# facebookresearch/vsc2022

Hardware: AMD Instinct MI355X
Metric: query-videos localized/sec @ 512-d SSCD (higher is better)
Workload: dtype fp32 results; int8 / fp16 MFMA pre-filters; 1 GPU; BASELINE configs[3]: full pipeline incl. score normalisation + TN localisation, 40000 query videos split over 1 GPU(s), 2000000 reference + 2000000 noise frames; query_videos_per_gpu=40000, query_frames_per_gpu=1000000, ref_frames=2000000, dim=512, global_k=48000000, candidates=1000000, pairs_localized=200000, matches=446939, hits=48000000, score_normalisation_in_step=True, parallelism=single GPU

## Files before the change

### vsc2022_amd/csrc/api_aux.hip

```cpp
#include "api_internal.h"

extern "C" {


struct DeviceCtx {
    hipStream_t stream = nullptr;
    hipStream_t own_stream = nullptr;
    Workspace ws;
    std::mutex mu;
};
static DeviceCtx* device_ctx(int device) {
    static std::mutex g_mu;
    static std::vector<DeviceCtx*> ctxs;
    std::lock_guard<std::mutex> lk(g_mu);
    if ((int)ctxs.size() <= device) ctxs.resize(device + 1, nullptr);
    if (!ctxs[device]) {
        DeviceCtx* c = new DeviceCtx();
        if (hipStreamCreateWithFlags(&c->own_stream, hipStreamNonBlocking) != hipSuccess) {
            delete c;
            return nullptr;
        }
        c->stream = c->own_stream;
        ctxs[device] = c;
    }
// ... 39 lines not shown
    VSC_TRY(check_device(device));
    VSC_HIP(hipSetDevice(device));
    DeviceCtx* c = device_ctx(device);
    if (!c) {
        set_error("vsc_pair_max: cannot create device context");
        return VSC_ERR_HIP;
    }
    std::lock_guard<std::mutex> lk(c->mu);
    Workspace& ws = c->ws;
    const void *di, *dj, *ds, *dq, *dr;
    VSC_TRY(to_device(hit_i, (size_t)n * 4, hits_mem, ws.hA[0], &di, c->stream));
    VSC_TRY(to_device(hit_j, (size_t)n * 4, hits_mem, ws.hA[1], &dj, c->stream));
    VSC_TRY(to_device(hit_s, (size_t)n * 4, hits_mem, ws.hA[2], &ds, c->stream));
    VSC_TRY(to_device(row2q, (size_t)nq_rows * 4, maps_mem, ws.maps0, &dq, c->stream));
    VSC_TRY(to_device(row2r, (size_t)nr_rows * 4, maps_mem, ws.maps1, &dr, c->stream));
    int32_t *oq = out_q, *orr = out_r;
    float* os = out_s;
    int64_t* of = out_first;
    const int64_t ocap = out_mem == VSC_MEM_HOST ? n : cap;
    if (out_mem == VSC_MEM_HOST) {
        VSC_TRY(ws.out[0].reserve((size_t)n * 4));
        VSC_TRY(ws.out[1].reserve((size_t)n * 4));
        VSC_TRY(ws.out[2].reserve((size_t)n * 4));
        VSC_TRY(ws.out[3].reserve((size_t)n * 8));
        oq = ws.out[0].as<int32_t>();
        orr = ws.out[1].as<int32_t>();
        os = ws.out[2].as<float>();
        of = ws.out[3].as<int64_t>();
    }
    int64_t np = 0;
    AuxTimer tm;
    tm.begin(0, c->stream);
    VSC_TRY(pair_max_device((const int32_t*)di, (const int32_t*)dj, (const float*)ds, n, (const int32_t*)dq,
                            (const int32_t*)dr, nq_rows, nr_rows, ws.w0, ws.w1, ws.w2, ws.w3, ws.tmp, ws.cnt, oq, orr, os, of,
                            ocap, &np, c->stream));
    tm.end(12.0 * (double)n + 20.0 * (double)np, c->stream);
    *n_pairs = np;
    if (out_mem == VSC_MEM_HOST) {
        if (np > cap) {
            set_error("vsc_pair_max: output capacity %lld < %lld pairs", (long long)cap, (long long)np);
            return VSC_ERR_CAPACITY;
        }
        VSC_HIP(hipMemcpyAsync(out_q, oq, (size_t)np * 4, hipMemcpyDeviceToHost, c->stream));
        VSC_HIP(hipMemcpyAsync(out_r, orr, (size_t)np * 4, hipMemcpyDeviceToHost, c->stream));
        VSC_HIP(hipMemcpyAsync(out_s, os, (size_t)np * 4, hipMemcpyDeviceToHost, c->stream));
        if (out_first) VSC_HIP(hipMemcpyAsync(out_first, of, (size_t)np * 8, hipMemcpyDeviceToHost, c->stream));
    }
    VSC_HIP(hipStreamSynchronize(c->stream));
    tm.collect();
    return VSC_OK;
}

int vsc_sort_hits(const int32_t* hit_i, const int32_t* hit_j, const float* hit_s, int64_t n, int hits_mem, int64_t max_row,
                  int64_t max_ref, int32_t* out_i, int32_t* out_j, float* out_s, int out_mem, int device) {
    if (n < 0 || (n > 0 && (!hit_i || !hit_j || !hit_s || !out_i || !out_j || !out_s))) {
        set_error("vsc_sort_hits: invalid argument");
        return VSC_ERR_INVALID;
    }
    if (n == 0) return VSC_OK;
    VSC_TRY(check_device(device));
    VSC_HIP(hipSetDevice(device));
    DeviceCtx* c = device_ctx(device);
    if (!c) {
        set_error("vsc_sort_hits: cannot create device context");
        return VSC_ERR_HIP;
    }
    std::lock_guard<std::mutex> lk(c->mu);
    Workspace& ws = c->ws;
    const void *di, *dj, *ds;
    VSC_TRY(to_device(hit_i, (size_t)n * 4, hits_mem, ws.hA[0], &di, c->stream));
    VSC_TRY(to_device(hit_j, (size_t)n * 4, hits_mem, ws.hA[1], &dj, c->stream));
    VSC_TRY(to_device(hit_s, (size_t)n * 4, hits_mem, ws.hA[2], &ds, c->stream));
    int32_t *oi = out_i, *oj = out_j;
    float* os = out_s;
    if (out_mem == VSC_MEM_HOST) {
        for (int k = 0; k < 3; ++k) VSC_TRY(ws.out[k].reserve((size_t)n * 4));
        oi = ws.out[0].as<int32_t>();
        oj = ws.out[1].as<int32_t>();
        os = ws.out[2].as<float>();
    }
    const int64_t all = (int64_t)1 << 31;
    int64_t m = 0;
    VSC_TRY(sort_hits_topk((const int32_t*)di, (const int32_t*)dj, (const float*)ds, n, n, max_row > 0 ? max_row : all,
                           max_ref > 0 ? max_ref : all, ws.w0, ws.w1, ws.w2, ws.w3, ws.tmp, oi, oj, os, 0, &m, c->stream));
    if (out_mem == VSC_MEM_HOST) {
        VSC_HIP(hipMemcpyAsync(out_i, oi, (size_t)n * 4, hipMemcpyDeviceToHost, c->stream));
        VSC_HIP(hipMemcpyAsync(out_j, oj, (size_t)n * 4, hipMemcpyDeviceToHost, c->stream));
        VSC_HIP(hipMemcpyAsync(out_s, os, (size_t)n * 4, hipMemcpyDeviceToHost, c->stream));
    }
    VSC_HIP(hipStreamSynchronize(c->stream));
    return VSC_OK;
}

int vsc_score_histogram(const float* scores, int64_t n, const int64_t* state, int shift, int64_t* hist, int device) {
    if (n < 0 || (n > 0 && !scores) || !state || !hist || (shift != 0 && shift != 8 && shift != 16 && shift != 24)) {
        set_error("vsc_score_histogram: invalid argument");
        return VSC_ERR_INVALID;
    }
    VSC_TRY(check_device(device));
    VSC_HIP(hipSetDevice(device));
    DeviceCtx* c = device_ctx(device);
    if (!c) {
        set_error("vsc_score_histogram: cannot create device context");
        return VSC_ERR_HIP;
    }
    std::lock_guard<std::mutex> lk(c->mu);
    VSC_TRY(launch_score_hist(scores, (long long)n, reinterpret_cast<const long long*>(state), shift,
                              reinterpret_cast<long long*>(hist), c->stream));
    if (c->stream == c->own_stream) VSC_HIP(hipStreamSynchronize(c->stream));
    return VSC_OK;
}

int vsc_score_pick(const int64_t* hist, int64_t* state, int shift, int device) {
    if (!hist || !state || (shift != 0 && shift != 8 && shift != 16 && shift != 24)) {
        set_error("vsc_score_pick: invalid argument");
        return VSC_ERR_INVALID;
    }
    VSC_TRY(check_device(device));
    VSC_HIP(hipSetDevice(device));
    DeviceCtx* c = device_ctx(device);
    if (!c) {
        set_error("vsc_score_pick: cannot create device context");
        return VSC_ERR_HIP;
    }
    std::lock_guard<std::mutex> lk(c->mu);
    VSC_TRY(launch_score_pick(reinterpret_cast<const long long*>(hist), reinterpret_cast<long long*>(state), shift, c->stream));
    if (c->stream == c->own_stream) VSC_HIP(hipStreamSynchronize(c->stream));
    return VSC_OK;
}

int vsc_filter_hits(const int32_t* hit_i, const int32_t* hit_j, const float* hit_s, int64_t n, float radius, int32_t* out_i,
                    int32_t* out_j, float* out_s, int64_t* n_out, int device) {
    if (n < 0 || !n_out || (n > 0 && (!hit_i || !hit_j || !hit_s || !out_i || !out_j || !out_s)) || !(radius == radius)) {
        set_error("vsc_filter_hits: invalid argument");
        return VSC_ERR_INVALID;
    }
    *n_out = 0;
    if (n == 0) return VSC_OK;
    VSC_TRY(check_device(device));
    VSC_HIP(hipSetDevice(device));
    DeviceCtx* c = device_ctx(device);
    if (!c) {
        set_error("vsc_filter_hits: cannot create device context");
        return VSC_ERR_HIP;
    }
    std::lock_guard<std::mutex> lk(c->mu);
    VSC_TRY(c->ws.cnt.reserve(sizeof(unsigned long long)));
    VSC_TRY(launch_filter_hits(hit_i, hit_j, hit_s, (long long)n, radius, out_i, out_j, out_s, c->ws.cnt.as<unsigned long long>(),
                               c->stream));
    unsigned long long kept = 0;
    VSC_HIP(hipMemcpyAsync(&kept, c->ws.cnt.p, sizeof(kept), hipMemcpyDeviceToHost, c->stream));
    VSC_HIP(hipStreamSynchronize(c->stream));
    *n_out = (int64_t)kept;
    return VSC_OK;
}

int vsc_argsort_scores(const float* scores, int64_t n, int mem, int32_t* perm, int perm_mem, int device) {
    if (n < 0 || (n > 0 && (!scores || !perm))) {
        set_error("vsc_argsort_scores: invalid argument");
        return VSC_ERR_INVALID;
    }
    if (n == 0) return VSC_OK;
    VSC_TRY(check_device(device));
    VSC_HIP(hipSetDevice(device));
    DeviceCtx* c = device_ctx(device);
    if (!c) {
        set_error("vsc_argsort_scores: cannot create device context");
// ... 416 lines not shown
```

### vsc2022_amd/csrc/kernels.h

```cpp
#pragma once
#include "vscmi_common.h"
#include "cand_list.h"

namespace vscmi {

struct SimThreshArgs {
    const float* Q; const float* R; int dpad; int nq; int i0; int nr; int tq; int tr;
    const float* radius; int32_t* out_i; int32_t* out_j; float* out_s;
    unsigned long long* counter; long long cap; int* overflow;
};
struct SimF16Args {
    const _Float16* Q; const _Float16* R;
    const float* qn; const float* rn;
    int dpadh; int nq; int i0; int nr; int tq; int tr;
    float c1, c2, c3;
    const float* radius; int32_t* out_i; int32_t* out_j;
    const float* row_thr;
    int seg_cap; int* seg_count; int64_t tail_base; long long tail_cap; int tail_shift; int* tail_fill; unsigned long long* tail_count;
    int* overflow;
};
constexpr int F16P_PANEL_ROWS = 128;
constexpr int F16P_COL_STEP = 512;
constexpr int F16P_MAX_DPADH = 512;
struct SimF16PArgs {
// ... 59 lines not shown
    unsigned long long* n_cand_total;
    const int* overflow;
};
struct SimKnnArgs {
    const float* Q; const float* R; int dpad; int nq; int nr; int tq; int tr; int nchunk; int k;
    float* part_s; int32_t* part_j;
    int no_first_tile_select;
};
struct KnnMergeArgs {
    const float* part_s; const int32_t* part_j; int nq; int nchunk; int k; float* out_s; int64_t* out_j; int l2;
};
struct ScoreMatArgs { const float* Q; const float* R; int dpad; int dim; int nq; int nr; int metric; float* S; };
struct MatThreshArgs {
    const float* S; int nq; int nr; int i0; const float* radius; int32_t* out_i; int32_t* out_j; float* out_s;
    unsigned long long* counter; long long cap; int* overflow;
};
struct MatKnnArgs { const float* S; int nq; int nr; int k; float* part_s; int32_t* part_j; };
struct SelectCtl {
    unsigned long long n; unsigned long long n_tmp; float radius; int overflow; int active;
    unsigned int prefix; unsigned int prefix_mask; unsigned long long rank; unsigned int hist[256];
    unsigned long long n_rethreshold;
    unsigned long long n_cand_total;
    unsigned long long n_tail;
};
struct TnPairArgs {
    const float* qfeat; const float* rfeat; const int64_t* q_off; const int64_t* r_off; int dpad;
    const int32_t* pair_q; const int32_t* pair_r; const int32_t* work; int n_work; vsc_tn_params prm;
    float bias; int max_lq; int lds_tile_floats; float* slab; int64_t slab_floats;
    int32_t* out_nbox; int32_t* out_boxes; float* out_boxmax;
    const float* sims_in; const int64_t* sims_off; const int32_t* sims_lq; const int32_t* sims_lr;
    char* state; int64_t state_bytes;
};
struct TnSimsArgs { const float* qfeat; const float* rfeat; int64_t qrow0, rrow0; int lq, lr, dpad; float bias; float* out; };

int launch_sim_thresh(const SimThreshArgs&, hipStream_t);
int launch_sim_f16(const SimF16Args&, hipStream_t);
int sim_f16_grid(int tq, int tr);
int launch_rescore(const RescoreArgs&, hipStream_t);
int launch_cand_count(const RescoreArgs&, int, unsigned long long*, hipStream_t);
int launch_cand_compact(const RescoreArgs&, int, uint32_t*, uint32_t*, unsigned long long*, hipStream_t);
int launch_rescore_dense(const RescoreArgs&, const uint32_t*, const uint32_t*, long long, hipStream_t,
                         const unsigned long long* n_dev = nullptr);
int launch_f16_screen(const ScreenArgs&, hipStream_t);
int sort_candidates_by_ref(uint32_t*, uint32_t*, uint32_t*, uint32_t*, int64_t, int64_t, DevBuf&, const uint32_t**,
                           const uint32_t**, hipStream_t);
void sim_f16p_plan(int64_t nq, int64_t nr, int* npanel, int* nsteps, int* slice, int* grid);
int launch_sim_f16p(const SimF16PArgs&, int grid, hipStream_t);
int launch_sim_i8p(const SimI8PArgs&, int grid, hipStream_t);
bool sim_i8p_pairs(int dpad8, int npanel, int nsteps, int slice, bool force);
int launch_quant_ref_frag(const float*, int, void*, float4*, int64_t, int64_t, int, const ExcludedDims&, const float*, hipStream_t);
int launch_col_sums(const float*, int64_t, int, double*, double*, hipStream_t);
int launch_row_center(const float*, int, int, const float*, float*, float*, hipStream_t);
int launch_dim_minmax(const float*, int64_t, int, unsigned*, unsigned*, hipStream_t);
int launch_meta_looseness(const float4*, int64_t, double*, hipStream_t);
int launch_quant_query_panels(const float*, int, int, int, void*, int, float4*, const int32_t*, const float*, float*,
                              const ExcludedDims&, hipStream_t);
int launch_row_absmax(const float*, int, int, const ExcludedDims&, float*, hipStream_t);
int launch_row_bias_thresholds(const float*, int, int, const float*, const float*, const ExcludedDims&, const float*, const float*, float*,
                               hipStream_t);
int sort_rows_by_threshold(const float*, int64_t, DevBuf&, DevBuf&, DevBuf&, DevBuf&, DevBuf&, const int32_t**, hipStream_t);
int argsort_scores_desc(const float*, int64_t, DevBuf&, DevBuf&, DevBuf&, DevBuf&, DevBuf&, const int32_t**, hipStream_t);
int launch_ctl_init(SelectCtl*, float, hipStream_t);
int launch_filter_hits(const int32_t*, const int32_t*, const float*, long long, float, int32_t*, int32_t*, float*, unsigned long long*,
                       hipStream_t);
int launch_score_hist(const float*, long long, const long long*, int, long long*, hipStream_t);
int launch_score_pick(const long long*, long long*, int, hipStream_t);
int launch_merge_topk(const float*, const long long*, long long, int, int, float*, long long*, hipStream_t);
int sort_rows_by_threshold_then_scale(const float*, const float*, int64_t, int, DevBuf&, DevBuf&, DevBuf&, DevBuf&, DevBuf&,
                                      const int32_t**, hipStream_t);
int launch_pack_half_frag(const float*, int64_t, int, _Float16*, float*, int64_t, int64_t, int, hipStream_t);
int launch_pack_half(const float*, int64_t, int, _Float16*, float*, int64_t, int, hipStream_t);
int launch_sim_knn(const SimKnnArgs&, hipStream_t);
int launch_knn_merge(const KnnMergeArgs&, hipStream_t);
int knn_from_hits(const int32_t*, const int32_t*, const float*, int64_t, int64_t, int, DevBuf&, DevBuf&, DevBuf&,
                  DevBuf&, DevBuf&, float*, int64_t*, hipStream_t);
int launch_knn_row_thr(const float*, int64_t, int, float*, int64_t, hipStream_t);
int launch_knn_seed_hits(const float*, const int64_t*, int64_t, int, int32_t*, int32_t*, float*, unsigned long long*, hipStream_t);
int launch_score_matrix(const ScoreMatArgs&, hipStream_t);
int launch_matrix_thresh(const MatThreshArgs&, hipStream_t);
int launch_matrix_knn(const MatKnnArgs&, hipStream_t);
int set_thresh_kernel_attrs();
int enqueue_rethreshold(SelectCtl*, int32_t*, int32_t*, float*, int32_t*, int32_t*, float*, unsigned long long, hipStream_t);
int sort_hits_topk(const int32_t*, const int32_t*, const float*, int64_t, int64_t, int64_t, int64_t, DevBuf&, DevBuf&,
                   DevBuf&, DevBuf&, DevBuf&, int32_t*, int32_t*, float*, int, int64_t*, hipStream_t);
int sort_hits_rowcol(const int32_t*, const int32_t*, const float*, int64_t, DevBuf&, DevBuf&, DevBuf&, DevBuf&,
                     DevBuf&, int32_t*, int32_t*, float*, int, hipStream_t);
int pair_max_device(const int32_t*, const int32_t*, const float*, int64_t, const int32_t*, const int32_t*, int64_t, int64_t,
                    DevBuf&, DevBuf&, DevBuf&, DevBuf&, DevBuf&, DevBuf&, int32_t*, int32_t*, float*, int64_t*,
                    int64_t, int64_t*, hipStream_t);
int launch_pack_rows(const float*, int64_t, int, float*, int64_t, int, hipStream_t);
int launch_row_normalize(const float*, int64_t, int, float*, hipStream_t);
size_t tn_state_bytes_host(int, int, int, int idx_bytes = 2);
int launch_tn_pairs(const TnPairArgs&, size_t, hipStream_t);
int launch_tn_sims(const TnSimsArgs&, hipStream_t);
int launch_encode_rows(const void*, bool, int64_t, int, _Float16*, float*, int64_t, int64_t, int, bool, int*, hipStream_t);
int launch_decode_rows(const _Float16*, int, bool, int64_t, int64_t, int64_t, float*, int, bool, hipStream_t);
int launch_unpack_rows(const float*, int, int64_t, int, float*, hipStream_t);
int launch_half_to_float(const _Float16*, int64_t, float*, hipStream_t);
int launch_score_matrix_h16(const ScoreMatArgs&, const _Float16*, int, bool, hipStream_t);
int launch_hits_mark(const unsigned long long*, unsigned long long*, hipStream_t);
int launch_hits_add_offset(int32_t*, const unsigned long long*, const unsigned long long*, long long, int, hipStream_t);
int launch_knn_parts_scatter(const float*, const int32_t*, int64_t, int, int, int, int, int, float*, int32_t*, hipStream_t);


}
```

### vsc2022_amd/csrc/radix.h

```cpp
#pragma once
#include "vscmi_common.h"

namespace vscmi {

constexpr int RADIX_ITEMS = 16;
constexpr int RADIX_TILE = 256 * RADIX_ITEMS;

template <class K>
__device__ __forceinline__ unsigned radix_digit(K key, int shift, bool desc) {
    if (desc) key = ~key;
    return (unsigned)(key >> shift) & 255u;
}

template <class K>
__global__ __launch_bounds__(256) void radix_hist_kernel(const K* __restrict__ keys, int64_t n, int shift, bool desc,
                                                         unsigned* __restrict__ hist, int ntiles) {
    __shared__ unsigned h[256];
    h[threadIdx.x] = 0;
    __syncthreads();
    const int64_t base = (int64_t)blockIdx.x * RADIX_TILE;
#pragma unroll 4
    for (int k = 0; k < RADIX_ITEMS; ++k) {
        const int64_t e = base + k * 256 + threadIdx.x;
        if (e < n) atomicAdd(&h[radix_digit(keys[e], shift, desc)], 1u);
    }
    __syncthreads();
    hist[(int64_t)threadIdx.x * ntiles + blockIdx.x] = h[threadIdx.x];
}

__global__ __launch_bounds__(256) void radix_scan_rows_kernel(unsigned* __restrict__ hist, int ntiles,
                                                              unsigned* __restrict__ totals) {
    __shared__ unsigned part[256];
    unsigned* row = hist + (int64_t)blockIdx.x * ntiles;
    const int per = (ntiles + 255) / 256;
    const int t0 = threadIdx.x * per;
    unsigned s = 0;
    for (int t = t0; t < min(ntiles, t0 + per); ++t) s += row[t];
    part[threadIdx.x] = s;
    __syncthreads();
    for (int off = 1; off < 256; off <<= 1) {
        const unsigned v = threadIdx.x >= off ? part[threadIdx.x - off] : 0u;
        __syncthreads();
        part[threadIdx.x] += v;
        __syncthreads();
    }
    unsigned run = threadIdx.x ? part[threadIdx.x - 1] : 0u;
    for (int t = t0; t < min(ntiles, t0 + per); ++t) {
        const unsigned c = row[t];
        row[t] = run;
        run += c;
    }
    if (threadIdx.x == 255) totals[blockIdx.x] = part[255];
}

__global__ __launch_bounds__(256) void radix_scan_totals_kernel(unsigned* __restrict__ totals) {
    __shared__ unsigned part[256];
    part[threadIdx.x] = totals[threadIdx.x];
    __syncthreads();
    for (int off = 1; off < 256; off <<= 1) {
        const unsigned v = threadIdx.x >= off ? part[threadIdx.x - off] : 0u;
        __syncthreads();
        part[threadIdx.x] += v;
        __syncthreads();
    }
    totals[threadIdx.x] = threadIdx.x ? part[threadIdx.x - 1] : 0u;
}

template <class K, class V>
__global__ __launch_bounds__(256) void radix_scatter_kernel(const K* __restrict__ keys_in, const V* __restrict__ vals_in,
                                                            K* __restrict__ keys_out, V* __restrict__ vals_out, int64_t n,
                                                            int shift, bool desc, const unsigned* __restrict__ hist,
                                                            const unsigned* __restrict__ totals, int ntiles) {
    __shared__ unsigned wcount[4][256];
    __shared__ unsigned dstart[256];
    __shared__ unsigned gbase[256];
    __shared__ K skey[RADIX_TILE];
    __shared__ V sval[RADIX_TILE];
    const int lane = threadIdx.x & 63, wave = threadIdx.x >> 6;
    for (int x = threadIdx.x; x < 4 * 256; x += 256) (&wcount[0][0])[x] = 0;
    gbase[threadIdx.x] = totals[threadIdx.x] + hist[(int64_t)threadIdx.x * ntiles + blockIdx.x];
    __syncthreads();
    const int64_t tile0 = (int64_t)blockIdx.x * RADIX_TILE;
    const int64_t base = tile0 + (int64_t)wave * (RADIX_ITEMS * 64);
    K key[RADIX_ITEMS];
    unsigned rank[RADIX_ITEMS];
#pragma unroll
    for (int k = 0; k < RADIX_ITEMS; ++k) {
        const int64_t e = base + k * 64 + lane;
        const bool valid = e < n;
        key[k] = valid ? keys_in[e] : (K)0;
        const unsigned d = radix_digit(key[k], shift, desc);
        unsigned long long peers = __ballot(valid);
#pragma unroll
        for (int b = 0; b < 8; ++b) {
            const unsigned long long m = __ballot((d >> b) & 1u);
            peers &= ((d >> b) & 1u) ? m : ~m;
        }
        const unsigned before = (unsigned)__popcll(peers & ((1ull << lane) - 1));
        unsigned c = 0;
        if (valid) c = wcount[wave][d];
        __builtin_amdgcn_wave_barrier();
        if (valid && before == 0) wcount[wave][d] = c + (unsigned)__popcll(peers);
        __builtin_amdgcn_wave_barrier();
        rank[k] = c + before;
    }
    __syncthreads();
    {
        const int d = threadIdx.x;
        unsigned run = 0;
#pragma unroll
        for (int w = 0; w < 4; ++w) {
            const unsigned c = wcount[w][d];
            wcount[w][d] = run;
            run += c;
        }
        dstart[d] = run;
    }
    __syncthreads();
    for (int off = 1; off < 256; off <<= 1) {
        const unsigned v = threadIdx.x >= off ? dstart[threadIdx.x - off] : 0u;
        __syncthreads();
        dstart[threadIdx.x] += v;
        __syncthreads();
    }
    const unsigned mine_incl = dstart[threadIdx.x];
    const unsigned prev_incl = threadIdx.x ? dstart[threadIdx.x - 1] : 0u;
    __syncthreads();
    dstart[threadIdx.x] = prev_incl;
    (void)mine_incl;
    __syncthreads();
#pragma unroll
    for (int k = 0; k < RADIX_ITEMS; ++k) {
        const int64_t e = base + k * 64 + lane;
        if (e < n) {
            const unsigned d = radix_digit(key[k], shift, desc);
            const unsigned slot = dstart[d] + wcount[wave][d] + rank[k];
            skey[slot] = key[k];
            sval[slot] = vals_in[e];
        }
    }
    __syncthreads();
    const int cnt = (int)min((int64_t)RADIX_TILE, n - tile0);
#pragma unroll 4
    for (int k = 0; k < RADIX_ITEMS; ++k) {
        const int slot = k * 256 + threadIdx.x;
        if (slot < cnt) {
            const K kk = skey[slot];
            const unsigned d = radix_digit(kk, shift, desc);
            const int64_t pos = (int64_t)gbase[d] + (slot - dstart[d]);
            keys_out[pos] = kk;
            vals_out[pos] = sval[slot];
        }
    }
}

inline size_t radix_tmp_bytes(int64_t n) {
    const int64_t ntiles = (n + RADIX_TILE - 1) / RADIX_TILE;
    return (size_t)(256 * ntiles + 256) * sizeof(unsigned);
}

template <class K, class V>
int radix_sort_pairs(K* keys_a, K* keys_b, V* vals_a, V* vals_b, int64_t n, int begin_bit, int end_bit, bool desc,
                     void* tmp, hipStream_t stream, int begin2 = 0, int end2 = 0) {
    if (n <= 0) return 0;
    if (n > 0xffffffffLL) {
        set_error("radix_sort_pairs: %lld entries exceed the 2^32 limit of the sort", (long long)n);
        return -1;
    }
    const int ntiles = (int)((n + RADIX_TILE - 1) / RADIX_TILE);
    unsigned* hist = reinterpret_cast<unsigned*>(tmp);
    unsigned* totals = hist + (size_t)256 * ntiles;
    int where = 0;
    for (int pass = 0;; ++pass) {
        const int n1 = (end_bit - begin_bit + 7) / 8;
        const int shift = pass < n1 ? begin_bit + 8 * pass : begin2 + 8 * (pass - n1);
        if (pass >= n1 && shift >= end2) break;
        const K* ki = where ? keys_b : keys_a;
        const V* vi = where ? vals_b : vals_a;
        K* ko = where ? keys_a : keys_b;
        V* vo = where ? vals_a : vals_b;
        hipLaunchKernelGGL((radix_hist_kernel<K>), dim3((unsigned)ntiles), dim3(256), 0, stream, ki, n, shift, desc, hist, ntiles);
        hipLaunchKernelGGL(radix_scan_rows_kernel, dim3(256), dim3(256), 0, stream, hist, ntiles, totals);
        hipLaunchKernelGGL(radix_scan_totals_kernel, dim3(1), dim3(256), 0, stream, totals);
        hipLaunchKernelGGL((radix_scatter_kernel<K, V>), dim3((unsigned)ntiles), dim3(256), 0, stream, ki, vi, ko, vo, n, shift,
                           desc, hist, totals, ntiles);
        if (hipGetLastError() != hipSuccess) return -1;
        where ^= 1;
    }
    return where;
}

}
```

### vsc2022_amd/csrc/sortpairs.hip

```cpp
#include <cfloat>
#include <cstring>
#include <utility>

#include "kernels.h"
#include "radix.h"

namespace vscmi {

__global__ __launch_bounds__(256) void pack_hits_kernel(const int32_t* i, const int32_t* j,
                                                        const float* s, int64_t n, uint64_t* key64,
                                                        uint32_t* key32) {
    const int64_t x = (int64_t)blockIdx.x * 256 + threadIdx.x;
    if (x >= n) return;
    key64[x] = ((uint64_t)(uint32_t)i[x] << 32) | (uint32_t)j[x];
    key32[x] = f2key(s[x]);
}

__global__ __launch_bounds__(256) void unpack_hits_kernel(const uint64_t* key64, const uint32_t* key32,
                                                          int64_t n, int32_t* i, int32_t* j, float* s,
                                                          int negate) {
    const int64_t x = (int64_t)blockIdx.x * 256 + threadIdx.x;
    if (x >= n) return;
    i[x] = (int32_t)(key64[x] >> 32);
    j[x] = (int32_t)(key64[x] & 0xffffffffu);
    const float v = key2f(key32[x]);
    s[x] = negate ? -v : v;
}

static inline unsigned grid_for(int64_t n) { return (unsigned)((n + 255) / 256); }

static int bits_for(uint64_t maxval) {
    int b = 1;
    while (b < 64 && (maxval >> b)) ++b;
    return b;
}

int sort_hits_topk(const int32_t* hi, const int32_t* hj, const float* hs, int64_t n, int64_t K,
                   int64_t max_i, int64_t max_j, DevBuf& w0, DevBuf& w1, DevBuf& w2, DevBuf& w3, DevBuf& tmp,
                   int32_t* out_i, int32_t* out_j, float* out_s, int negate, int64_t* n_out,
                   hipStream_t stream) {
    const int64_t m = n < K ? n : K;
    *n_out = m;
    if (n <= 0) return VSC_OK;
    VSC_TRY(w0.reserve(sizeof(uint64_t) * n));
    VSC_TRY(w1.reserve(sizeof(uint64_t) * n));
    VSC_TRY(w2.reserve(sizeof(uint32_t) * n));
    VSC_TRY(w3.reserve(sizeof(uint32_t) * n));
    uint64_t* k64a = w0.as<uint64_t>();
    uint64_t* k64b = w1.as<uint64_t>();
    uint32_t* k32a = w2.as<uint32_t>();
    uint32_t* k32b = w3.as<uint32_t>();
    hipLaunchKernelGGL(pack_hits_kernel, dim3(grid_for(n)), dim3(256), 0, stream, hi, hj, hs, n, k64a, k32a);
    VSC_HIP(hipGetLastError());
    const int end_bit = 32 + bits_for((uint64_t)(max_i > 0 ? max_i : 1));
    VSC_TRY(tmp.reserve(radix_tmp_bytes(n)));
    int w = radix_sort_pairs<uint64_t, uint32_t>(k64a, k64b, k32a, k32b, n, 0, max_j > 0 ? bits_for((uint64_t)max_j) : 32, false,
                                                 tmp.p, stream, 32, end_bit);
    if (w < 0) { set_error("radix sort launch failed"); return VSC_ERR_HIP; }
    if (w) { std::swap(k64a, k64b); std::swap(k32a, k32b); }
    w = radix_sort_pairs<uint32_t, uint64_t>(k32a, k32b, k64a, k64b, n, 0, 32, true, tmp.p, stream);
    if (w < 0) { set_error("radix sort launch failed"); return VSC_ERR_HIP; }
    if (w) { std::swap(k64a, k64b); std::swap(k32a, k32b); }
    hipLaunchKernelGGL(unpack_hits_kernel, dim3(grid_for(m)), dim3(256), 0, stream, k64a, k32a, m, out_i, out_j, out_s, negate);
    VSC_HIP(hipGetLastError());
    return VSC_OK;
}

__global__ __launch_bounds__(256) void thr_keys_kernel(const float* __restrict__ thr, int n, uint32_t* __restrict__ keys,
                                                       int32_t* __restrict__ vals) {
    const int x = blockIdx.x * 256 + threadIdx.x;
    if (x >= n) return;
    keys[x] = f2key(thr[x]);
    vals[x] = x;
}

int sort_rows_by_threshold(const float* thr, int64_t n, DevBuf& w0, DevBuf& w1, DevBuf& w2, DevBuf& w3, DevBuf& tmp,
                           const int32_t** perm, hipStream_t stream) {
    *perm = nullptr;
    if (n <= 0) return VSC_OK;
    VSC_TRY(w0.reserve(sizeof(uint32_t) * n));
    VSC_TRY(w1.reserve(sizeof(uint32_t) * n));
    VSC_TRY(w2.reserve(sizeof(int32_t) * n));
    VSC_TRY(w3.reserve(sizeof(int32_t) * n));
    VSC_TRY(tmp.reserve(radix_tmp_bytes(n)));
    uint32_t *ka = w0.as<uint32_t>(), *kb = w1.as<uint32_t>();
    int32_t *va = w2.as<int32_t>(), *vb = w3.as<int32_t>();
    hipLaunchKernelGGL(thr_keys_kernel, dim3(grid_for(n)), dim3(256), 0, stream, thr, (int)n, ka, va);
    VSC_HIP(hipGetLastError());
    const int w = radix_sort_pairs<uint32_t, int32_t>(ka, kb, va, vb, n, 0, 32, false, tmp.p, stream);
    if (w < 0) { set_error("radix sort launch failed"); return VSC_ERR_HIP; }
    *perm = w ? vb : va;
    return VSC_OK;
}

__global__ __launch_bounds__(256) void score_keys_kernel(const float* __restrict__ s, long long n, uint32_t* __restrict__ keys,
                                                         int32_t* __restrict__ vals) {
    const long long x = (long long)blockIdx.x * 256 + threadIdx.x;
    if (x >= n) return;
    keys[x] = f2key(s[x] + 0.0f);
    vals[x] = (int32_t)x;
}

int argsort_scores_desc(const float* s, int64_t n, DevBuf& w0, DevBuf& w1, DevBuf& w2, DevBuf& w3, DevBuf& tmp,
                        const int32_t** perm, hipStream_t stream) {
    *perm = nullptr;
    if (n <= 0) return VSC_OK;
    VSC_TRY(w0.reserve(sizeof(uint32_t) * n));
    VSC_TRY(w1.reserve(sizeof(uint32_t) * n));
    VSC_TRY(w2.reserve(sizeof(int32_t) * n));
    VSC_TRY(w3.reserve(sizeof(int32_t) * n));
    VSC_TRY(tmp.reserve(radix_tmp_bytes(n)));
    uint32_t *ka = w0.as<uint32_t>(), *kb = w1.as<uint32_t>();
    int32_t *va = w2.as<int32_t>(), *vb = w3.as<int32_t>();
    hipLaunchKernelGGL(score_keys_kernel, dim3(grid_for(n)), dim3(256), 0, stream, s, (long long)n, ka, va);
    VSC_HIP(hipGetLastError());
    const int w = radix_sort_pairs<uint32_t, int32_t>(ka, kb, va, vb, n, 0, 32, true, tmp.p, stream);
    if (w < 0) { set_error("radix sort launch failed"); return VSC_ERR_HIP; }
    *perm = w ? vb : va;
    return VSC_OK;
}

__global__ __launch_bounds__(256) void group_scale_keys_kernel(const int32_t* __restrict__ perm, const float* __restrict__ scale,
                                                               int n, int group_shift, uint32_t* __restrict__ keys) {
    const int p = blockIdx.x * 256 + threadIdx.x;
    if (p >= n) return;
    keys[p] = ((uint32_t)(p >> group_shift) << 20) | (f2key(scale[perm[p]]) >> 12);
}

__global__ __launch_bounds__(1024) void group_scale_rank_kernel(const int32_t* __restrict__ perm, const float* __restrict__ scale, int n,
                                                                int group_shift, int32_t* __restrict__ out) {
    __shared__ uint32_t key[1024];
    const int G = 1 << group_shift;
    const int base = blockIdx.x << group_shift;
    const int cnt = min(G, n - base);
    const int t = threadIdx.x;
    int32_t row = 0;
    uint32_t mine = 0;
    if (t < cnt) {
        row = perm[base + t];
        mine = f2key(scale[row]) >> 12;
        key[t] = mine;
    }
    __syncthreads();
    if (t >= cnt) return;
    int rank = 0;
    for (int f = 0; f < cnt; ++f) {
// ... 183 lines not shown
                  DevBuf& w1, DevBuf& w2, DevBuf& w3, DevBuf& tmp, float* out_s, int64_t* out_j,
                  hipStream_t stream) {
    const int64_t nn = n > 0 ? n : 1;
    VSC_TRY(w0.reserve(sizeof(uint64_t) * nn));
    VSC_TRY(w1.reserve(sizeof(uint64_t) * nn));
    VSC_TRY(w2.reserve(sizeof(uint32_t) * nn));
    VSC_TRY(w3.reserve(sizeof(uint32_t) * nn));
    uint64_t* ka = w0.as<uint64_t>();
    uint64_t* kb = w1.as<uint64_t>();
    uint32_t* ra = w2.as<uint32_t>();
    uint32_t* rb = w3.as<uint32_t>();
    if (n > 0) {
        hipLaunchKernelGGL(knn_keys_kernel, dim3(grid_for(n)), dim3(256), 0, stream, hi, hs, n, ka);
        VSC_HIP(hipGetLastError());
        VSC_HIP(hipMemcpyAsync(ra, hj, (size_t)n * 4, hipMemcpyDeviceToDevice, stream));
        const int end_bit = 32 + bits_for((uint64_t)(nq > 0 ? nq : 1));
        VSC_TRY(tmp.reserve(radix_tmp_bytes(n)));
        int w = radix_sort_pairs<uint32_t, uint64_t>(ra, rb, ka, kb, n, 0, 32, false, tmp.p, stream);
        if (w < 0) { set_error("radix sort launch failed"); return VSC_ERR_HIP; }
        if (w) { std::swap(ka, kb); std::swap(ra, rb); }
        w = radix_sort_pairs<uint64_t, uint32_t>(ka, kb, ra, rb, n, 0, end_bit, false, tmp.p, stream);
        if (w < 0) { set_error("radix sort launch failed"); return VSC_ERR_HIP; }
        if (w) { std::swap(ka, kb); std::swap(ra, rb); }
    }
    hipLaunchKernelGGL(knn_cut_kernel, dim3(grid_for(nq * k)), dim3(256), 0, stream, ka, ra, n, nq, k, out_s, out_j);
    VSC_HIP(hipGetLastError());
    return VSC_OK;
}

__global__ __launch_bounds__(256) void knn_seed_hits_kernel(const float* __restrict__ knn_s, const int64_t* __restrict__ knn_j,
                                                            int64_t n, int k, int32_t* __restrict__ hi, int32_t* __restrict__ hj,
                                                            float* __restrict__ hs, unsigned long long* __restrict__ counter) {
    const int64_t x = (int64_t)blockIdx.x * 256 + threadIdx.x;
    const bool have = x < n && knn_j[x] >= 0;
    const unsigned long long m = __ballot(have);
    if (m == 0ull) return;
    const int lane = threadIdx.x & 63;
    unsigned long long base = 0;
    if (lane == __ffsll((long long)m) - 1) base = atomicAdd(counter, (unsigned long long)__popcll(m));
    base = __shfl(base, __ffsll((long long)m) - 1);
    if (have) {
        const unsigned long long p = base + __popcll(m & ((1ull << lane) - 1));
        hi[p] = (int32_t)(x / k);
        hj[p] = (int32_t)knn_j[x];
        hs[p] = knn_s[x];
    }
}

int launch_knn_seed_hits(const float* knn_s, const int64_t* knn_j, int64_t nq, int k, int32_t* hi, int32_t* hj, float* hs,
                         unsigned long long* counter, hipStream_t stream) {
    const int64_t n = nq * k;
    if (n <= 0) return VSC_OK;
    hipLaunchKernelGGL(knn_seed_hits_kernel, dim3(grid_for(n)), dim3(256), 0, stream, knn_s, knn_j, n, k, hi, hj, hs, counter);
    VSC_HIP(hipGetLastError());
    return VSC_OK;
}

__global__ __launch_bounds__(256) void knn_row_thr_kernel(const float* knn_s, int64_t nq, int k, float* row_thr,
                                                          int64_t rows) {
    const int64_t x = (int64_t)blockIdx.x * 256 + threadIdx.x;
    if (x >= rows) return;
    row_thr[x] = x < nq ? knn_s[x * k + (k - 1)] : INFINITY;
}

int launch_knn_row_thr(const float* knn_s, int64_t nq, int k, float* row_thr, int64_t rows, hipStream_t stream) {
    if (rows <= 0) return VSC_OK;
    hipLaunchKernelGGL(knn_row_thr_kernel, dim3(grid_for(rows)), dim3(256), 0, stream, knn_s, nq, k, row_thr, rows);
    VSC_HIP(hipGetLastError());
    return VSC_OK;
}

int sort_hits_rowcol(const int32_t* hi, const int32_t* hj, const float* hs, int64_t n, DevBuf& w0,
                     DevBuf& w1, DevBuf& w2, DevBuf& w3, DevBuf& tmp, int32_t* out_i, int32_t* out_j,
                     float* out_s, int negate, hipStream_t stream) {
    if (n <= 0) return VSC_OK;
    VSC_TRY(w0.reserve(sizeof(uint64_t) * n));
    VSC_TRY(w1.reserve(sizeof(uint64_t) * n));
    VSC_TRY(w2.reserve(sizeof(uint32_t) * n));
    VSC_TRY(w3.reserve(sizeof(uint32_t) * n));
    uint64_t* k64a = w0.as<uint64_t>();
    uint64_t* k64b = w1.as<uint64_t>();
    uint32_t* k32a = w2.as<uint32_t>();
    uint32_t* k32b = w3.as<uint32_t>();
    hipLaunchKernelGGL(pack_hits_kernel, dim3(grid_for(n)), dim3(256), 0, stream, hi, hj, hs, n, k64a, k32a);
    VSC_HIP(hipGetLastError());
    VSC_TRY(tmp.reserve(radix_tmp_bytes(n)));
    const int w = radix_sort_pairs<uint64_t, uint32_t>(k64a, k64b, k32a, k32b, n, 0, 64, false, tmp.p, stream);
    if (w < 0) { set_error("radix sort launch failed"); return VSC_ERR_HIP; }
    if (w) { std::swap(k64a, k64b); std::swap(k32a, k32b); }
    hipLaunchKernelGGL(unpack_hits_kernel, dim3(grid_for(n)), dim3(256), 0, stream, k64a, k32a, n, out_i, out_j, out_s, negate);
    VSC_HIP(hipGetLastError());
    return VSC_OK;
}

}
```

Measured before the change: 19890 query-videos/s.

## Rework radix sort with variable-width digits, 512-thread tiles and self-scan

Replaces the fixed 8-bit, 256-thread LSD radix sort with up to 11-bit digits planned evenly across each bit range. This reduces the number of passes, which use 512-thread blocks and dynamic LDS. Small inputs skip the separate scan kernel by having each scatter block sum histogram rows itself, and the totals-scan kernel is folded into the scatter via a block scan. It also adds a tie_zeros option to the hit sort that keeps -0.0 scores distinct from +0.0 by tagging a key bit. The trade-off is larger histograms, more LDS per block and a per-thread loop over digit bits.

```diff
diff --git a/vsc2022_amd/csrc/api_aux.hip b/vsc2022_amd/csrc/api_aux.hip
--- a/vsc2022_amd/csrc/api_aux.hip
+++ b/vsc2022_amd/csrc/api_aux.hip
@@ -145,7 +145,8 @@
     const int64_t all = (int64_t)1 << 31;
     int64_t m = 0;
     VSC_TRY(sort_hits_topk((const int32_t*)di, (const int32_t*)dj, (const float*)ds, n, n, max_row > 0 ? max_row : all,
-                           max_ref > 0 ? max_ref : all, ws.w0, ws.w1, ws.w2, ws.w3, ws.tmp, oi, oj, os, 0, &m, c->stream));
+                           max_ref > 0 ? max_ref : all, ws.w0, ws.w1, ws.w2, ws.w3, ws.tmp, oi, oj, os, 0, &m, c->stream,
+                           1));
     if (out_mem == VSC_MEM_HOST) {
         VSC_HIP(hipMemcpyAsync(out_i, oi, (size_t)n * 4, hipMemcpyDeviceToHost, c->stream));
         VSC_HIP(hipMemcpyAsync(out_j, oj, (size_t)n * 4, hipMemcpyDeviceToHost, c->stream));
diff --git a/vsc2022_amd/csrc/kernels.h b/vsc2022_amd/csrc/kernels.h
--- a/vsc2022_amd/csrc/kernels.h
+++ b/vsc2022_amd/csrc/kernels.h
@@ -165,7 +165,7 @@
 int set_thresh_kernel_attrs();
 int enqueue_rethreshold(SelectCtl*, int32_t*, int32_t*, float*, int32_t*, int32_t*, float*, unsigned long long, hipStream_t);
 int sort_hits_topk(const int32_t*, const int32_t*, const float*, int64_t, int64_t, int64_t, int64_t, DevBuf&, DevBuf&,
-                   DevBuf&, DevBuf&, DevBuf&, int32_t*, int32_t*, float*, int, int64_t*, hipStream_t);
+                   DevBuf&, DevBuf&, DevBuf&, int32_t*, int32_t*, float*, int, int64_t*, hipStream_t, int tie_zeros = 0);
 int sort_hits_rowcol(const int32_t*, const int32_t*, const float*, int64_t, DevBuf&, DevBuf&, DevBuf&, DevBuf&,
                      DevBuf&, int32_t*, int32_t*, float*, int, hipStream_t);
 int pair_max_device(const int32_t*, const int32_t*, const float*, int64_t, const int32_t*, const int32_t*, int64_t, int64_t,
diff --git a/vsc2022_amd/csrc/radix.h b/vsc2022_amd/csrc/radix.h
--- a/vsc2022_amd/csrc/radix.h
+++ b/vsc2022_amd/csrc/radix.h
@@ -3,29 +3,50 @@
 
 namespace vscmi {
 
-constexpr int RADIX_ITEMS = 16;
-constexpr int RADIX_TILE = 256 * RADIX_ITEMS;
+constexpr int RADIX_THREADS = 512;
+constexpr int RADIX_WAVES = RADIX_THREADS / 64;
+constexpr int RADIX_MAX_BITS = 11;
+constexpr int RADIX_MAX_BINS = 1 << RADIX_MAX_BITS;
+constexpr int RADIX_SELF_SCAN_TILES = 32;
+
+constexpr int RADIX_TILE = 16 * RADIX_THREADS;
+
+template <class K, class V>
+struct RadixShape {
+    static constexpr int ITEMS = RADIX_TILE / RADIX_THREADS;
+    static constexpr int TILE = RADIX_TILE;
+    static constexpr int XBYTES = sizeof(K) > sizeof(V) ? sizeof(K) : sizeof(V);
+    static constexpr int CNT_BYTES = RADIX_WAVES * RADIX_MAX_BINS * 4;
+    static constexpr int BUF_BYTES = TILE * XBYTES > CNT_BYTES ? TILE * XBYTES : CNT_BYTES;
+    static constexpr int LDS_BYTES = BUF_BYTES + RADIX_MAX_BINS * 4 + 2 * RADIX_WAVES * 4;
+};
+
+inline int& radix_max_digit_bits() {
+    static int bits = RADIX_MAX_BITS;
+    return bits;
+}
 
 template <class K>
-__device__ __forceinline__ unsigned radix_digit(K key, int shift, bool desc) {
+__device__ __forceinline__ unsigned radix_digit(K key, int shift, unsigned mask, bool desc) {
     if (desc) key = ~key;
-    return (unsigned)(key >> shift) & 255u;
-}
-
-template <class K>
-__global__ __launch_bounds__(256) void radix_hist_kernel(const K* __restrict__ keys, int64_t n, int shift, bool desc,
-                                                         unsigned* __restrict__ hist, int ntiles) {
-    __shared__ unsigned h[256];
-    h[threadIdx.x] = 0;
-    __syncthreads();
-    const int64_t base = (int64_t)blockIdx.x * RADIX_TILE;
-#pragma unroll 4
-    for (int k = 0; k < RADIX_ITEMS; ++k) {
-        const int64_t e = base + k * 256 + threadIdx.x;
-        if (e < n) atomicAdd(&h[radix_digit(keys[e], shift, desc)], 1u);
-    }
-    __syncthreads();
-    hist[(int64_t)threadIdx.x * ntiles + blockIdx.x] = h[threadIdx.x];
+    return (unsigned)(key >> shift) & mask;
+}
+
+template <class K, int TILE>
+__global__ __launch_bounds__(RADIX_THREADS) void radix_hist_kernel(const K* __restrict__ keys, int64_t n, int shift,
+                                                                   unsigned mask, bool desc, unsigned* __restrict__ hist,
+                                                                   int ntiles) {
+    __shared__ unsigned h[RADIX_MAX_BINS];
+    for (unsigned d = threadIdx.x; d <= mask; d += RADIX_THREADS) h[d] = 0;
+    __syncthreads();
+    const int64_t base = (int64_t)blockIdx.x * TILE;
+#pragma unroll 8
+    for (int k = 0; k < TILE / RADIX_THREADS; ++k) {
+        const int64_t e = base + k * RADIX_THREADS + threadIdx.x;
+        if (e < n) atomicAdd(&h[radix_digit(keys[e], shift, mask, desc)], 1u);
+    }
+    __syncthreads();
+    for (unsigned d = threadIdx.x; d <= mask; d += RADIX_THREADS) hist[(int64_t)d * ntiles + blockIdx.x] = h[d];
 }
 
 __global__ __launch_bounds__(256) void radix_scan_rows_kernel(unsigned* __restrict__ hist, int ntiles,
@@ -53,46 +74,83 @@
     if (threadIdx.x == 255) totals[blockIdx.x] = part[255];
 }
 
-__global__ __launch_bounds__(256) void radix_scan_totals_kernel(unsigned* __restrict__ totals) {
-    __shared__ unsigned part[256];
-    part[threadIdx.x] = totals[threadIdx.x];
-    __syncthreads();
-    for (int off = 1; off < 256; off <<= 1) {
-        const unsigned v = threadIdx.x >= off ? part[threadIdx.x - off] : 0u;
-        __syncthreads();
-        part[threadIdx.x] += v;
-        __syncthreads();
-    }
-    totals[threadIdx.x] = threadIdx.x ? part[threadIdx.x - 1] : 0u;
+__device__ __forceinline__ void radix_block_scan4(const unsigned v[4], unsigned out[4], unsigned* wsum) {
+    const int lane = threadIdx.x & 63, wave = threadIdx.x >> 6;
+    const unsigned s = v[0] + v[1] + v[2] + v[3];
+    unsigned inc = s;
+#pragma unroll
+    for (int off = 1; off < 64; off <<= 1) {
+        const unsigned u = (unsigned)__shfl_up((int)inc, off);
+        if (lane >= off) inc += u;
+    }
+    if (lane == 63) wsum[wave] = inc;
+    __syncthreads();
+    unsigned run = inc - s;
+    for (int w = 0; w < wave; ++w) run += wsum[w];
+    out[0] = run;
+    out[1] = run + v[0];
+    out[2] = out[1] + v[1];
+    out[3] = out[2] + v[2];
 }
 
 template <class K, class V>
-__global__ __launch_bounds__(256) void radix_scatter_kernel(const K* __restrict__ keys_in, const V* __restrict__ vals_in,
-                                                            K* __restrict__ keys_out, V* __restrict__ vals_out, int64_t n,
-                                                            int shift, bool desc, const unsigned* __restrict__ hist,
-                                                            const unsigned* __restrict__ totals, int ntiles) {
-    __shared__ unsigned wcount[4][256];
-    __shared__ unsigned dstart[256];
-    __shared__ unsigned gbase[256];
-    __shared__ K skey[RADIX_TILE];
-    __shared__ V sval[RADIX_TILE];
+__global__ __launch_bounds__(RADIX_THREADS) __attribute__((amdgpu_waves_per_eu(4, 4))) void radix_scatter_kernel(const K* __restrict__ keys_in, const V* __restrict__ vals_in,
+                                                                      K* __restrict__ keys_out, V* __restrict__ vals_out, int64_t n,
+                                                                      int shift, int bits, bool desc,
+                                                                      const unsigned* __restrict__ hist,
+                                                                      const unsigned* __restrict__ totals, int ntiles,
+                                                                      int self_scan) {
+    typedef RadixShape<K, V> S;
+    constexpr int ITEMS = S::ITEMS, TILE = S::TILE;
+    extern __shared__ __attribute__((aligned(16))) unsigned char radix_smem[];
+    unsigned(*wcount)[RADIX_MAX_BINS] = reinterpret_cast<unsigned(*)[RADIX_MAX_BINS]>(radix_smem);
+    K* skey = reinterpret_cast<K*>(radix_smem);
+    V* sval = reinterpret_cast<V*>(radix_smem);
+    unsigned* dstart = reinterpret_cast<unsigned*>(radix_smem + S::BUF_BYTES);
+    unsigned* wsum = dstart + RADIX_MAX_BINS;
     const int lane = threadIdx.x & 63, wave = threadIdx.x >> 6;
-    for (int x = threadIdx.x; x < 4 * 256; x += 256) (&wcount[0][0])[x] = 0;
-    gbase[threadIdx.x] = totals[threadIdx.x] + hist[(int64_t)threadIdx.x * ntiles + blockIdx.x];
-    __syncthreads();
-    const int64_t tile0 = (int64_t)blockIdx.x * RADIX_TILE;
-    const int64_t base = tile0 + (int64_t)wave * (RADIX_ITEMS * 64);
-    K key[RADIX_ITEMS];
-    unsigned rank[RADIX_ITEMS];
-#pragma unroll
-    for (int k = 0; k < RADIX_ITEMS; ++k) {
-        const int64_t e = base + k * 64 + lane;
-        const bool valid = e < n;
-        key[k] = valid ? keys_in[e] : (K)0;
-        const unsigned d = radix_digit(key[k], shift, desc);
+    const unsigned mask = (1u << bits) - 1u;
+    const int nbins = 1 << bits;
+    {
+        uint4* z = reinterpret_cast<uint4*>(radix_smem);
+        for (int x = threadIdx.x; x < S::CNT_BYTES / 16; x += RADIX_THREADS) z[x] = make_uint4(0, 0, 0, 0);
+    }
+    unsigned gpre[4], gtot[4];
+#pragma unroll
+    for (int q = 0; q < 4; ++q) {
+        const int d = 4 * threadIdx.x + q;
+        gpre[q] = 0;
+        gtot[q] = 0;
+        if (d < nbins) {
+            const unsigned* row = hist + (int64_t)d * ntiles;
+            if (self_scan) {
+                for (int t = 0; t < ntiles; ++t) {
+                    const unsigned c = row[t];
+                    gtot[q] += c;
+                    if (t < (int)blockIdx.x) gpre[q] += c;
+                }
+            } else {
+                gpre[q] = row[blockIdx.x];
+                gtot[q] = totals[d];
+            }
+        }
+    }
+    __syncthreads();
+    const int64_t tile0 = (int64_t)blockIdx.x * TILE;
+    const int cnt = (int)min((int64_t)TILE, n - tile0);
+    const int base = wave * (ITEMS * 64) + lane;
+    keys_in += tile0;
+    vals_in += tile0;
+    K key[ITEMS];
+    unsigned rank[ITEMS];
+#pragma unroll
+    for (int k = 0; k < ITEMS; ++k) key[k] = base + k * 64 < cnt ? keys_in[base + k * 64] : (K)0;
+#pragma unroll
+    for (int k = 0; k < ITEMS; ++k) {
+        const bool valid = base + k * 64 < cnt;
+        const unsigned d = radix_digit(key[k], shift, mask, desc);
         unsigned long long peers = __ballot(valid);
-#pragma unroll
-        for (int b = 0; b < 8; ++b) {
+        for (int b = 0; b < bits; ++b) {
             const unsigned long long m = __ballot((d >> b) & 1u);
             peers &= ((d >> b) & 1u) ? m : ~m;
         }
@@ -105,85 +163,112 @@
         rank[k] = c + before;
     }
     __syncthreads();
+    unsigned tot[4] = {0, 0, 0, 0};
     {
-        const int d = threadIdx.x;
-        unsigned run = 0;
-#pragma unroll
-        for (int w = 0; w < 4; ++w) {
-            const unsigned c = wcount[w][d];
-            wcount[w][d] = run;
-            run += c;
-        }
-        dstart[d] = run;
-    }
-    __syncthreads();
-    for (int off = 1; off < 256; off <<= 1) {
-        const unsigned v = threadIdx.x >= off ? dstart[threadIdx.x - off] : 0u;
-        __syncthreads();
-        dstart[threadIdx.x] += v;
-        __syncthreads();
-    }
-    const unsigned mine_incl = dstart[threadIdx.x];
-    const unsigned prev_incl = threadIdx.x ? dstart[threadIdx.x - 1] : 0u;
-    __syncthreads();
-    dstart[threadIdx.x] = prev_incl;
-    (void)mine_incl;
-    __syncthreads();
-#pragma unroll
-    for (int k = 0; k < RADIX_ITEMS; ++k) {
-        const int64_t e = base + k * 64 + lane;
-        if (e < n) {
-            const unsigned d = radix_digit(key[k], shift, desc);
-            const unsigned slot = dstart[d] + wcount[wave][d] + rank[k];
-            skey[slot] = key[k];
-            sval[slot] = vals_in[e];
-        }
-    }
-    __syncthreads();
-    const int cnt = (int)min((int64_t)RADIX_TILE, n - tile0);
-#pragma unroll 4
-    for (int k = 0; k < RADIX_ITEMS; ++k) {
-        const int slot = k * 256 + threadIdx.x;
+        uint4* col = reinterpret_cast<uint4*>(&wcount[0][4 * threadIdx.x]);
+#pragma unroll
+        for (int w = 0; w < RADIX_WAVES; ++w) {
+            const uint4 c = col[w * (RADIX_MAX_BINS / 4)];
+            col[w * (RADIX_MAX_BINS / 4)] = make_uint4(tot[0], tot[1], tot[2], tot[3]);
+            tot[0] += c.x; tot[1] += c.y; tot[2] += c.z; tot[3] += c.w;
+        }
+    }
+    unsigned tstart[4], gstart[4];
+    radix_block_scan4(tot, tstart, wsum);
+    radix_block_scan4(gtot, gstart, wsum + RADIX_WAVES);
+    *reinterpret_cast<uint4*>(&dstart[4 * threadIdx.x]) = make_uint4(tstart[0], tstart[1], tstart[2], tstart[3]);
+    __syncthreads();
+#pragma unroll
+    for (int k = 0; k < ITEMS; ++k) {
+        const unsigned d = radix_digit(key[k], shift, mask, desc);
+        rank[k] += dstart[d] + wcount[wave][d];
+    }
+    __syncthreads();
+#pragma unroll
+    for (int q = 0; q < 4; ++q) dstart[4 * threadIdx.x + q] = gstart[q] + gpre[q] - tstart[q];
+#pragma unroll
+    for (int k = 0; k < ITEMS; ++k)
+        if (base + k * 64 < cnt) skey[rank[k]] = key[k];
+    __syncthreads();
+    unsigned pos[ITEMS];
+#pragma unroll
+    for (int k = 0; k < ITEMS; ++k) {
+        const int slot = k * RADIX_THREADS + threadIdx.x;
         if (slot < cnt) {
             const K kk = skey[slot];
-            const unsigned d = radix_digit(kk, shift, desc);
-            const int64_t pos = (int64_t)gbase[d] + (slot - dstart[d]);
-            keys_out[pos] = kk;
-            vals_out[pos] = sval[slot];
-        }
+            pos[k] = dstart[radix_digit(kk, shift, mask, desc)] + (unsigned)slot;
+            keys_out[pos[k]] = kk;
+        }
+    }
+    __syncthreads();
+#pragma unroll
+    for (int k = 0; k < ITEMS; ++k)
+        if (base + k * 64 < cnt) sval[rank[k]] = vals_in[base + k * 64];
+    __syncthreads();
+#pragma unroll
+    for (int k = 0; k < ITEMS; ++k) {
+        const int slot = k * RADIX_THREADS + threadIdx.x;
+        if (slot < cnt) vals_out[pos[k]] = sval[slot];
     }
 }
 
 inline size_t radix_tmp_bytes(int64_t n) {
     const int64_t ntiles = (n + RADIX_TILE - 1) / RADIX_TILE;
-    return (size_t)(256 * ntiles + 256) * sizeof(unsigned);
+    return (size_t)(RADIX_MAX_BINS * ntiles + RADIX_MAX_BINS) * sizeof(unsigned);
+}
+
+inline int radix_plan_range(int begin_bit, int end_bit, int* shift, int* width, int np) {
+    const int bits = end_bit - begin_bit;
+    if (bits <= 0) return np;
+    const int maxw = radix_max_digit_bits();
+    const int passes = (bits + maxw - 1) / maxw;
+    int at = begin_bit;
+    for (int p = 0; p < passes; ++p) {
+        const int w = bits / passes + (p < bits % passes ? 1 : 0);
+        shift[np] = at;
+        width[np] = w;
+        at += w;
+        ++np;
+    }
+    return np;
 }
 
 template <class K, class V>
 int radix_sort_pairs(K* keys_a, K* keys_b, V* vals_a, V* vals_b, int64_t n, int begin_bit, int end_bit, bool desc,
                      void* tmp, hipStream_t stream, int begin2 = 0, int end2 = 0) {
+    typedef RadixShape<K, V> S;
     if (n <= 0) return 0;
     if (n > 0xffffffffLL) {
         set_error("radix_sort_pairs: %lld entries exceed the 2^32 limit of the sort", (long long)n);
         return -1;
     }
-    const int ntiles = (int)((n + RADIX_TILE - 1) / RADIX_TILE);
+    static PerDeviceOnce once;
+    if (once.first()) {
+        if (hipFuncSetAttribute(reinterpret_cast<const void*>(&radix_scatter_kernel<K, V>),
+                                hipFuncAttributeMaxDynamicSharedMemorySize, S::LDS_BYTES) != hipSuccess)
+            return -1;
+        once.commit();
+    }
+    int shift[16], width[16];
+    int np = radix_plan_range(begin_bit, end_bit, shift, width, 0);
+    np = radix_plan_range(begin2, end2, shift, width, np);
+    const int ntiles = (int)((n + S::TILE - 1) / S::TILE);
+    const int self_scan = ntiles <= RADIX_SELF_SCAN_TILES;
     unsigned* hist = reinterpret_cast<unsigned*>(tmp);
-    unsigned* totals = hist + (size_t)256 * ntiles;
     int where = 0;
-    for (int pass = 0;; ++pass) {
-        const int n1 = (end_bit - begin_bit + 7) / 8;
-        const int shift = pass < n1 ? begin_bit + 8 * pass : begin2 + 8 * (pass - n1);
-        if (pass >= n1 && shift >= end2) break;
+    for (int pass = 0; pass < np; ++pass) {
+        const int nbins = 1 << width[pass];
+        unsigned* totals = hist + (size_t)nbins * ntiles;
         const K* ki = where ? keys_b : keys_a;
         const V* vi = where ? vals_b : vals_a;
         K* ko = where ? keys_a : keys_b;
         V* vo = where ? vals_a : vals_b;
-        hipLaunchKernelGGL((radix_hist_kernel<K>), dim3((unsigned)ntiles), dim3(256), 0, stream, ki, n, shift, desc, hist, ntiles);
-        hipLaunchKernelGGL(radix_scan_rows_kernel, dim3(256), dim3(256), 0, stream, hist, ntiles, totals);
-        hipLaunchKernelGGL(radix_scan_totals_kernel, dim3(1), dim3(256), 0, stream, totals);
-        hipLaunchKernelGGL((radix_scatter_kernel<K, V>), dim3((unsigned)ntiles), dim3(256), 0, stream, ki, vi, ko, vo, n, shift,
-                           desc, hist, totals, ntiles);
+        hipLaunchKernelGGL((radix_hist_kernel<K, S::TILE>), dim3((unsigned)ntiles), dim3(RADIX_THREADS), 0, stream, ki, n,
+                           shift[pass], (unsigned)nbins - 1u, desc, hist, ntiles);
+        if (!self_scan)
+            hipLaunchKernelGGL(radix_scan_rows_kernel, dim3((unsigned)nbins), dim3(256), 0, stream, hist, ntiles, totals);
+        hipLaunchKernelGGL((radix_scatter_kernel<K, V>), dim3((unsigned)ntiles), dim3(RADIX_THREADS), S::LDS_BYTES, stream, ki,
+                           vi, ko, vo, n, shift[pass], width[pass], desc, hist, totals, ntiles, self_scan);
         if (hipGetLastError() != hipSuccess) return -1;
         where ^= 1;
     }
diff --git a/vsc2022_amd/csrc/sortpairs.hip b/vsc2022_amd/csrc/sortpairs.hip
--- a/vsc2022_amd/csrc/sortpairs.hip
+++ b/vsc2022_amd/csrc/sortpairs.hip
@@ -9,21 +9,23 @@
 
 __global__ __launch_bounds__(256) void pack_hits_kernel(const int32_t* i, const int32_t* j,
                                                         const float* s, int64_t n, uint64_t* key64,
-                                                        uint32_t* key32) {
-    const int64_t x = (int64_t)blockIdx.x * 256 + threadIdx.x;
-    if (x >= n) return;
-    key64[x] = ((uint64_t)(uint32_t)i[x] << 32) | (uint32_t)j[x];
-    key32[x] = f2key(s[x]);
+                                                        uint32_t* key32, int tie_zeros) {
+    const int64_t x = (int64_t)blockIdx.x * 256 + threadIdx.x;
+    if (x >= n) return;
+    const bool neg_zero = tie_zeros && __float_as_uint(s[x]) == 0x80000000u;
+    key64[x] = ((uint64_t)(uint32_t)i[x] << 32) | (uint32_t)j[x] | (neg_zero ? 1ull << 63 : 0ull);
+    key32[x] = f2key(neg_zero ? 0.0f : s[x]);
 }
 
 __global__ __launch_bounds__(256) void unpack_hits_kernel(const uint64_t* key64, const uint32_t* key32,
                                                           int64_t n, int32_t* i, int32_t* j, float* s,
-                                                          int negate) {
-    const int64_t x = (int64_t)blockIdx.x * 256 + threadIdx.x;
-    if (x >= n) return;
-    i[x] = (int32_t)(key64[x] >> 32);
+                                                          int negate, int tie_zeros) {
+    const int64_t x = (int64_t)blockIdx.x * 256 + threadIdx.x;
+    if (x >= n) return;
+    const bool neg_zero = tie_zeros && (key64[x] >> 63);
+    i[x] = (int32_t)((key64[x] >> 32) & (tie_zeros ? 0x7fffffffu : 0xffffffffu));
     j[x] = (int32_t)(key64[x] & 0xffffffffu);
-    const float v = key2f(key32[x]);
+    const float v = neg_zero ? -0.0f : key2f(key32[x]);
     s[x] = negate ? -v : v;
 }
 
@@ -38,7 +40,7 @@
 int sort_hits_topk(const int32_t* hi, const int32_t* hj, const float* hs, int64_t n, int64_t K,
                    int64_t max_i, int64_t max_j, DevBuf& w0, DevBuf& w1, DevBuf& w2, DevBuf& w3, DevBuf& tmp,
                    int32_t* out_i, int32_t* out_j, float* out_s, int negate, int64_t* n_out,
-                   hipStream_t stream) {
+                   hipStream_t stream, int tie_zeros) {
     const int64_t m = n < K ? n : K;
     *n_out = m;
     if (n <= 0) return VSC_OK;
@@ -50,9 +52,9 @@
     uint64_t* k64b = w1.as<uint64_t>();
     uint32_t* k32a = w2.as<uint32_t>();
     uint32_t* k32b = w3.as<uint32_t>();
-    hipLaunchKernelGGL(pack_hits_kernel, dim3(grid_for(n)), dim3(256), 0, stream, hi, hj, hs, n, k64a, k32a);
-    VSC_HIP(hipGetLastError());
-    const int end_bit = 32 + bits_for((uint64_t)(max_i > 0 ? max_i : 1));
+    hipLaunchKernelGGL(pack_hits_kernel, dim3(grid_for(n)), dim3(256), 0, stream, hi, hj, hs, n, k64a, k32a, tie_zeros);
+    VSC_HIP(hipGetLastError());
+    const int end_bit = std::min(63, 32 + bits_for((uint64_t)(max_i > 0 ? max_i : 1)));
     VSC_TRY(tmp.reserve(radix_tmp_bytes(n)));
     int w = radix_sort_pairs<uint64_t, uint32_t>(k64a, k64b, k32a, k32b, n, 0, max_j > 0 ? bits_for((uint64_t)max_j) : 32, false,
                                                  tmp.p, stream, 32, end_bit);
@@ -61,7 +63,7 @@
     w = radix_sort_pairs<uint32_t, uint64_t>(k32a, k32b, k64a, k64b, n, 0, 32, true, tmp.p, stream);
     if (w < 0) { set_error("radix sort launch failed"); return VSC_ERR_HIP; }
     if (w) { std::swap(k64a, k64b); std::swap(k32a, k32b); }
-    hipLaunchKernelGGL(unpack_hits_kernel, dim3(grid_for(m)), dim3(256), 0, stream, k64a, k32a, m, out_i, out_j, out_s, negate);
+    hipLaunchKernelGGL(unpack_hits_kernel, dim3(grid_for(m)), dim3(256), 0, stream, k64a, k32a, m, out_i, out_j, out_s, negate, tie_zeros);
     VSC_HIP(hipGetLastError());
     return VSC_OK;
 }
@@ -411,15 +413,15 @@
     uint64_t* k64b = w1.as<uint64_t>();
     uint32_t* k32a = w2.as<uint32_t>();
     uint32_t* k32b = w3.as<uint32_t>();
-    hipLaunchKernelGGL(pack_hits_kernel, dim3(grid_for(n)), dim3(256), 0, stream, hi, hj, hs, n, k64a, k32a);
+    hipLaunchKernelGGL(pack_hits_kernel, dim3(grid_for(n)), dim3(256), 0, stream, hi, hj, hs, n, k64a, k32a, 0);
     VSC_HIP(hipGetLastError());
     VSC_TRY(tmp.reserve(radix_tmp_bytes(n)));
     const int w = radix_sort_pairs<uint64_t, uint32_t>(k64a, k64b, k32a, k32b, n, 0, 64, false, tmp.p, stream);
     if (w < 0) { set_error("radix sort launch failed"); return VSC_ERR_HIP; }
     if (w) { std::swap(k64a, k64b); std::swap(k32a, k32b); }
-    hipLaunchKernelGGL(unpack_hits_kernel, dim3(grid_for(n)), dim3(256), 0, stream, k64a, k32a, n, out_i, out_j, out_s, negate);
-    VSC_HIP(hipGetLastError());
-    return VSC_OK;
-}
-
-}
+    hipLaunchKernelGGL(unpack_hits_kernel, dim3(grid_for(n)), dim3(256), 0, stream, k64a, k32a, n, out_i, out_j, out_s, negate, 0);
+    VSC_HIP(hipGetLastError());
+    return VSC_OK;
+}
+
+}
```

Result: no change. 19950 query-videos/s, median of 6 (+0.3%).
